# ebartrum/lightning_gan_zoo

Measured on AMD Instinct MI355X. Metric: images/sec (G+D step) at 64x64 bs=128/GPU, higher is better.
Workload: dtype f32; 1 GPU; dc_gan synthetic 64x64 bs=128/GPU, one optimizer cycle of 2 batches (Lightning alternation + toggle), reference optimizer, fp32; key=dc_gan_bs128, global_batch=128, parallelism=dp1, images_counted=2*bs*n_gpus per step (every batch of the cycle)

## Files before the change

### lightning_gan_zoo_amd/csrc/gz_igemm2.h

```cpp
#pragma once
#include "gz_igemm_core.h"

namespace gz {

constexpr int STAGES2 = 3;
constexpr uint32_t SOFF_OOB = 0x80000000u;

template <int WM_, int WN_, int TN_, int OCC_, int TM_ = 4>
struct TileCfg2 {
    static constexpr int WM = WM_, WN = WN_, TM = TM_, TN = TN_, OCC = OCC_;
    static constexpr int BM = WM * TM * 32, BN = WN * TN * 32;
    static_assert(WM * WN == 4, "4 wavefronts per workgroup, one per SIMD");
};

template <int BN>
struct MContigB2 {
    static_assert(BN == 64 || BN == 128 || BN == 256, "piece mapping");
    using Params = typename MContigLoader<BN>::Params;
    static constexpr int LD = BN, ROWS = BK;
    static constexpr int PIECES = BK * BN / 256 / 4;
    static constexpr int RPP = 256 / BN;
    __amdgpu_buffer_rsrc_t rsrc;
    uint32_t voff, ldb;
    int wave;
    __device__ __forceinline__ void init(const Params& p, int tile, int y, int tid) {
        rsrc = make_rsrc(p.base + (long long)y * p.batch_stride, (uint32_t)p.K * p.ld * 4u);
        const int lane = tid & 63;
        wave = __builtin_amdgcn_readfirstlane(tid >> 6);
        const int f = lane * 4, r = f / BN, col = f % BN;
        const int n = tile * BN + col;
        ldb = (uint32_t)p.ld * 4u;
        voff = n < p.MN ? (uint32_t)(r * p.ld + n) * 4u : OOB;
    }
    __device__ __forceinline__ void issue_piece(int kc, float* stage, int p, bool live) {
        const int piece = wave * PIECES + p;
        bload_lds16(rsrc, stage + piece * 256, voff, live ? (uint32_t)(kc * BK + piece * RPP) * ldb : SOFF_OOB);
    }
};

template <int BM>
struct ConvDgA2 {
    static_assert(BM == 256 || BM == 512, "whole 256-pixel pieces per LDS row");
    using Params = typename ConvDgALoader<BM, 4, 4, 2, 1>::Params;
    static constexpr int PPR = BM / 256;
    static constexpr int LD = BM + 4, ROWS = BK / 2, PIECES = 2 * PPR;
    static constexpr int ZERO_COL = BM;
    static constexpr bool ROWSHARE = true;
    __amdgpu_buffer_rsrc_t rsrc;
    uint32_t voff[2 * PPR];
    int wave, K, OHW, shift_half1;
    __device__ __forceinline__ void init(const Params& p, int tile, int phase, int tid) {
        const ConvShape& s = p.s;
        rsrc = make_rsrc(p.y, (uint32_t)s.N * s.K * s.OH * s.OW * 4u);
        const int lane = tid & 63;
        wave = __builtin_amdgcn_readfirstlane(tid >> 6);
        K = s.K; OHW = s.OH * s.OW;
        const int py = phase / 2, px = phase % 2;
        shift_half1 = (px + 1) / 2 - 1;
#pragma unroll
        for (int hb = 0; hb < PPR; ++hb) {
            const uint32_t m = (uint32_t)tile * BM + hb * 256 + lane * 4;
            const bool m_ok = m < (uint32_t)s.N * p.AH * p.AW;
            const uint32_t n = fdiv(m, p.div_ahw);
            const uint32_t pix = m - n * (uint32_t)(p.AH * p.AW);
            const uint32_t a = fdiv(pix, p.div_aw);
            const uint32_t b = pix - a * (uint32_t)p.AW;
#pragma unroll
            for (int ty = 0; ty < 2; ++ty) {
                const int oy = (int)a + (py + 1) / 2 - ty;
                const bool ok = m_ok && (unsigned)oy < (unsigned)s.OH;
                voff[ty * PPR + hb] = ok ? (n * (uint32_t)(s.K * OHW) + (uint32_t)(oy * s.OW) + b) * 4u : OOB;
            }
        }
    }
    __device__ __forceinline__ int frag_shift(int half) const { return half ? shift_half1 : shift_half1 + 1; }
    __device__ __forceinline__ void issue_piece(int kc, float* stage, int p, bool live) {
        const int kol = kc * (BK / 4) + wave;
        bload_lds16(rsrc, stage + (wave * 2 + p / PPR) * LD + (p % PPR) * 256, voff[p],
                    (live && kol < K) ? (uint32_t)kol * (uint32_t)OHW * 4u : SOFF_OOB);
    }
};

template <int BM, int OWC>
struct ConvFwdA2 {
    static_assert(BM == 256 && BM % OWC == 0 && OWC >= 2, "piece mapping");
    using Params = typename ConvFwdALoader<BM, 4, 4, 2, 1>::Params;
    static constexpr int LD = BM, ROWS = BK / 2, PIECES = 2;
    static constexpr int OW_C = OWC;
    static constexpr int EXTRA = (6 * OWC + 4 + 3) & ~3;
    static constexpr bool FWDROWS = true;
    __amdgpu_buffer_rsrc_t rsrc;
    uint32_t voff[2];
    int wave, HW, C;
    __device__ __forceinline__ void init(const Params& p, int tile, int y, int tid) {
        const ConvShape& s = p.s;
        rsrc = make_rsrc(p.x, (uint32_t)(s.N * s.C * s.H * s.W) * 4u);
        const int lane = tid & 63;
        wave = __builtin_amdgcn_readfirstlane(tid >> 6);
        HW = s.H * s.W; C = s.C;
#pragma unroll
        for (int q = 0; q < 2; ++q) {
            const int f = ((wave * 2 + q) * 64 + lane) * 4;
            const int seg = f / (8 * OWC), rem = f - seg * 8 * OWC;
            const int ky = rem / (2 * OWC), col = rem - ky * 2 * OWC;
            const uint32_t m = (uint32_t)tile * BM + seg * OWC;
            const bool m_ok = m < (uint32_t)s.N * s.OH * s.OW;
            const uint32_t n = fdiv(m, p.div_ohw);
            const uint32_t oy = fdiv(m - n * (uint32_t)(s.OH * s.OW), p.div_ow);
            const int iy = (int)oy * 2 - 1 + ky;
            const bool ok = m_ok && (unsigned)iy < (unsigned)s.H;
            voff[q] = ok ? (n * (uint32_t)(s.C * HW) + (uint32_t)(iy * s.W + col)) * 4u : OOB;
        }
    }
    static constexpr int ZERO = ROWS * LD;
    __device__ __forceinline__ void frag(int m_local, int half, int& even, int& odd) const {
        const int seg = m_local / OWC, ox = m_local - seg * OWC;
        const int base = seg * 8 * OWC + 2 * ox - 1 + half;
        even = (half == 0 && ox == 0) ? ZERO : base;
        odd = (half == 1 && ox == OWC - 1) ? ZERO : base + 2;
    }
    __device__ __forceinline__ void issue_piece(int kc, float* stage, int p, bool live) {
        bload_lds16(rsrc, stage + (wave * 2 + p) * 256, voff[p], (live && kc < C) ? (uint32_t)kc * (uint32_t)HW * 4u : SOFF_OOB);
    }
};

template <class Geo_>
struct TapGatherA2 {
    using Geo = Geo_;
    using Params = typename Geo::Params;
    static constexpr int BM = Geo::BM, LD = BM, ROWS = BK;
    static constexpr int G = BM / 64;
    static constexpr int PIECES = BK * G / 4;
    Geo geo;
    __amdgpu_buffer_rsrc_t rsrc;
    uint32_t vbase[G], veff[G];
    typename Geo::Pix pix[G];
    int wave, blocks, last_tap, last_kc, cb;
    uint32_t tap_soff;
    __device__ __forceinline__ void init(const Params& p, int tile, int y, int tid) {
        rsrc = geo.init(p, y);
        const int lane = tid & 63;
        wave = __builtin_amdgcn_readfirstlane(tid >> 6);
        blocks = round_bk(geo.chans) / BK;
        last_tap = -1; last_kc = -1; cb = 0; tap_soff = 0;
#pragma unroll
        for (int g = 0; g < G; ++g) {
            vbase[g] = geo.locate(p, (uint32_t)tile * BM + g * 64 + lane, pix[g]);
            veff[g] = OOB;
        }
    }
    __device__ __forceinline__ void issue_piece(int kc, float* stage, int p, bool live) {
        if (p == 0) {
            int tap = last_tap;
            if (kc == last_kc + 1 && last_kc >= 0) {
                cb += BK;
                if (cb >= blocks * BK) { cb = 0; ++tap; }
            } else {
                tap = kc / blocks;
// ... 125 lines not shown
template <int BM>
struct PlaneA2 {
    static_assert(BM % 256 == 0, "whole 256-pixel pieces per LDS row");
    struct Params {
        const float* base;
        int CH, HW, M;
        FastDiv div_hw;
    };
    static constexpr int LD = BM, ROWS = BK;
    static constexpr int PPR = BM / 256;
    static constexpr int PIECES = BK * PPR / 4;
    __amdgpu_buffer_rsrc_t rsrc;
    uint32_t voff[PPR], plane;
    int wave, CH;
    __device__ __forceinline__ void init(const Params& p, int tile, int y, int tid) {
        rsrc = make_rsrc(p.base, (uint32_t)(p.M / p.HW) * (uint32_t)p.CH * (uint32_t)p.HW * 4u);
        const int lane = tid & 63;
        wave = __builtin_amdgcn_readfirstlane(tid >> 6);
        CH = p.CH;
        plane = (uint32_t)p.HW * 4u;
#pragma unroll
        for (int g = 0; g < PPR; ++g) {
            const uint32_t m = (uint32_t)tile * BM + g * 256 + 4 * lane;
            const uint32_t n = fdiv(m, p.div_hw);
            voff[g] = m < (uint32_t)p.M ? (n * (uint32_t)(p.CH * p.HW) + (m - n * (uint32_t)p.HW)) * 4u : OOB;
        }
    }
    __device__ __forceinline__ void issue_piece(int kc, float* stage, int p, bool live) {
        const int row = wave * 4 + p / PPR, g = p % PPR;
        const int c = kc * BK + row;
        bload_lds16(rsrc, stage + row * LD + g * 256, voff[g], (live && c < CH) ? (uint32_t)c * plane : SOFF_OOB);
    }
};

#ifdef GZ2_STAMPS
__device__ unsigned long long gz2_stamps[8192 * 8];
#define GZ2_STAMP(var) const unsigned long long var = __builtin_amdgcn_s_memtime()
#else
#define GZ2_STAMP(var)
#endif

#ifndef GZ2_EXP_NOP
#define GZ2_NOP ""
#else
#define GZ2_NOP "s_nop 1\n\t"
#endif
template <int OFF>
__device__ __forceinline__ float lds_rd(uint32_t byte_addr) {
    float v;
    asm volatile("ds_read_b32 %0, %1 offset:%2" : "=v"(v) : "v"(byte_addr), "n"(OFF) : "memory");
    return v;
}
__device__ __forceinline__ void mfma_row(f32x16 (&c)[4], float a, const float (&b)[4]) {
    asm volatile(GZ2_NOP
                 "v_mfma_f32_32x32x2_f32 %0, %5, %4, %0\n\t"
                 "v_mfma_f32_32x32x2_f32 %1, %6, %4, %1\n\t"
                 "v_mfma_f32_32x32x2_f32 %2, %7, %4, %2\n\t"
                 "v_mfma_f32_32x32x2_f32 %3, %8, %4, %3"
                 : "+a"(c[0]), "+a"(c[1]), "+a"(c[2]), "+a"(c[3])
                 : "v"(a), "v"(b[0]), "v"(b[1]), "v"(b[2]), "v"(b[3]));
}
__device__ __forceinline__ void mfma_row(f32x16 (&c)[2], float a, const float (&b)[2]) {
    asm volatile(GZ2_NOP
                 "v_mfma_f32_32x32x2_f32 %0, %3, %2, %0\n\t"
                 "v_mfma_f32_32x32x2_f32 %1, %4, %2, %1"
                 : "+a"(c[0]), "+a"(c[1])
                 : "v"(a), "v"(b[0]), "v"(b[1]));
}
__device__ __forceinline__ void mfma_row(f32x16 (&c)[1], float a, const float (&b)[1]) {
    asm volatile(GZ2_NOP
                 "v_mfma_f32_32x32x2_f32 %0, %2, %1, %0"
                 : "+a"(c[0])
                 : "v"(a), "v"(b[0]));
}
__device__ __forceinline__ void mfma_one(f32x16& c, float a, float b) {
    asm volatile(GZ2_NOP
                 "v_mfma_f32_32x32x2_f32 %0, %2, %1, %0"
                 : "+a"(c)
                 : "v"(a), "v"(b));
}
__device__ __forceinline__ void mfma_row_mn(f32x16 (&c)[4], float a, const float (&b)[4]) {
    asm volatile(GZ2_NOP
                 "v_mfma_f32_32x32x2_f32 %0, %4, %5, %0\n\t"
                 "v_mfma_f32_32x32x2_f32 %1, %4, %6, %1\n\t"
                 "v_mfma_f32_32x32x2_f32 %2, %4, %7, %2\n\t"
                 "v_mfma_f32_32x32x2_f32 %3, %4, %8, %3"
                 : "+a"(c[0]), "+a"(c[1]), "+a"(c[2]), "+a"(c[3])
                 : "v"(a), "v"(b[0]), "v"(b[1]), "v"(b[2]), "v"(b[3]));
}
__device__ __forceinline__ void mfma_row_mn(f32x16 (&c)[2], float a, const float (&b)[2]) {
    asm volatile(GZ2_NOP
                 "v_mfma_f32_32x32x2_f32 %0, %2, %3, %0\n\t"
                 "v_mfma_f32_32x32x2_f32 %1, %2, %4, %1"
                 : "+a"(c[0]), "+a"(c[1])
                 : "v"(a), "v"(b[0]), "v"(b[1]));
}
__device__ __forceinline__ void lgkm_done(float (&a)[4], float (&b)[4]) {
    asm volatile("s_waitcnt lgkmcnt(0)" : "+v"(a[0]), "+v"(a[1]), "+v"(a[2]), "+v"(a[3]), "+v"(b[0]), "+v"(b[1]), "+v"(b[2]), "+v"(b[3]));
}
__device__ __forceinline__ void lgkm_done(float (&a)[4], float (&b)[2]) {
    asm volatile("s_waitcnt lgkmcnt(0)" : "+v"(a[0]), "+v"(a[1]), "+v"(a[2]), "+v"(a[3]), "+v"(b[0]), "+v"(b[1]));
}
__device__ __forceinline__ void lgkm_done(float (&a)[2], float (&b)[4]) {
    asm volatile("s_waitcnt lgkmcnt(0)" : "+v"(a[0]), "+v"(a[1]), "+v"(b[0]), "+v"(b[1]), "+v"(b[2]), "+v"(b[3]));
}
__device__ __forceinline__ void lgkm_done(float (&a)[4], float (&b)[1]) {
    asm volatile("s_waitcnt lgkmcnt(0)" : "+v"(a[0]), "+v"(a[1]), "+v"(a[2]), "+v"(a[3]), "+v"(b[0]));
}

template <class AL, class = void>
struct a_extra_of { static constexpr int value = 0; };
template <class AL>
struct a_extra_of<AL, std::void_t<decltype(AL::EXTRA)>> { static constexpr int value = AL::EXTRA; };
template <class AL>
constexpr int igemm2_a_extra() { return a_extra_of<AL>::value; }
template <class AL, class = void>
struct fwd_ow_of { static constexpr int value = 1; };
template <class AL>
struct fwd_ow_of<AL, std::void_t<decltype(AL::OW_C)>> { static constexpr int value = AL::OW_C; };
template <class AL>
constexpr int fwd_ow() { return fwd_ow_of<AL>::value; }

template <class AL>
constexpr int mode_count_of() {
    if constexpr (is_dualmode<AL>::value) return AL::MODES;
    else return 1;
}
template <class AL>
constexpr bool mode_plain_of(int m, int S) {
    if constexpr (is_dualmode<AL>::value) return AL::step_plain(m, S);
    else return false;
}
template <class AL>
constexpr unsigned mode_mask_of(int m, int S) {
    if constexpr (is_dualmode<AL>::value) return AL::step_mask(m, S);
    else return 0xFu;
}
template <class AL>
constexpr int ksteps_of() {
    if constexpr (is_dualmode<AL>::value) return AL::KSTEPS;
    else return BK / 2;
}
template <class AL>
constexpr int step_arow_of(int m, int S) {
    if constexpr (is_dualmode<AL>::value) return AL::step_arow(m, S);
    else return S;
}
template <class AL>
constexpr int step_brow_of(int m, int S) {
    if constexpr (is_dualmode<AL>::value) return AL::step_brow(m, S);
    else return 2 * S;
}

template <class Cfg, class AL, class BL, int KG>
constexpr int igemm2_ring_floats() {
    return ((STAGES2 * (AL::ROWS * AL::LD + igemm2_a_extra<AL>() + BL::ROWS * BL::LD) + 63) / 64) * 64;
}

template <class Cfg, class AL, class BL, class Epi, int KG = 1>
__global__ __launch_bounds__(NT * KG, KG == 1 ? Cfg::OCC : 2) void igemm2_kernel(typename AL::Params pa, typename BL::Params pb,
                                                                              typename Epi::Params pe, GridMap gm) {
    constexpr int LDA = AL::LD, LDB = BL::LD;
    constexpr int TM = Cfg::TM, TN = Cfg::TN;
    static_assert((TM == 4 || (TM == 2 && is_dualmode<AL>::value)) && (TN == 1 || TN == 2 || TN == 4),
                  "fragment registers of the hand-ordered k-step");
    static_assert(KG == 1 || (KG == 2 && TN <= 2), "two wave groups: the parked accumulators must fit the LDS");
    constexpr bool RS = is_rowshare<AL>::value;
    constexpr bool FR = is_fwdrows<AL>::value;
    constexpr bool DM = is_dualmode<AL>::value;
    static_assert(!DM || (RS && KG == 1 && (TN == 2 || TN == 4)), "multi-mode: row-shared loader, phases in the accumulator blocks");
    constexpr int A_EXTRA = igemm2_a_extra<AL>();
    constexpr int A_ELEMS = AL::ROWS * LDA + A_EXTRA, B_ELEMS = BL::ROWS * LDB;
    constexpr int STAGE = A_ELEMS + B_ELEMS;
    constexpr int PAD = 16;
    extern __shared__ __attribute__((aligned(16))) float smem2[];
    const int kg = KG == 1 ? 0 : __builtin_amdgcn_readfirstlane((int)threadIdx.x >> 8);
    float* const ring = smem2 + PAD + kg * igemm2_ring_floats<Cfg, AL, BL, KG>();
    GZ2_STAMP(st0);
#ifdef GZ2_STAMPS
    const unsigned long long sr0 = __builtin_amdgcn_s_memrealtime();
    unsigned long long st1 = st0, st2 = st0;
#endif

    const int tid = KG == 1 ? (int)threadIdx.x : ((int)threadIdx.x & (NT - 1));
    const int nwg = gridDim.x;
    int bid = blockIdx.x;
    if (gm.stagger > 0 && bid < 512 && blockIdx.z == 0) {
        const unsigned hw = __builtin_amdgcn_s_getreg(((4 - 1) << 11) | (16 << 6) | 4);
        if (hw & 1u) {
            const unsigned long long t_end = __builtin_amdgcn_s_memtime() + (unsigned long long)gm.stagger;
            while (__builtin_amdgcn_s_memtime() < t_end) __builtin_amdgcn_s_sleep(64);
        }
    }
    int y;
    if (gm.var_chunks) {
        const int tiles = gm.tiles_m * gm.tiles_n;
        y = gm.phase_order[bid / tiles];
        bid %= tiles;
    } else {
        if (!gm.no_swizzle) {
            const int q = nwg >> 3, rr = nwg & 7, x = bid & 7, i = bid >> 3;
            bid = (x < rr ? x * (q + 1) : rr * (q + 1) + (x - rr) * q) + i;
        }
        y = bid % gm.ny;
        bid /= gm.ny;
    }
    const int tile_n = bid % gm.tiles_n;
    const int tile_m = bid / gm.tiles_n;
    const int z = blockIdx.z;
    const int kcA = z * gm.chunks_per_split;
    const int kcB = min(gm.var_chunks ? gm.phase_chunks[y] : gm.chunks, kcA + gm.chunks_per_split);
    if (gm.slab && gm.var_chunks && kcA >= kcB) return;
    int kc0 = kcA, kc1 = kcB, kend = kcB;
    if constexpr (KG == 2) {
        const int h = (kcB - kcA + 1) >> 1;
        kc0 = kcA + kg * h;
        kend = kc0 + h;
        kc1 = min(kcB, kend);
    }

    AL al;
    BL bl;
    al.init(pa, tile_m, y, tid);
    bl.init(pb, tile_n, y, tid);

    f32x16 acc[TM][TN];
#pragma unroll
    for (int i = 0; i < TM; ++i)
#pragma unroll
        for (int j = 0; j < TN; ++j)
#pragma unroll
            for (int r = 0; r < 16; ++r) acc[i][j][r] = 0.f;

    const int lane = tid & 63, wave = __builtin_amdgcn_readfirstlane(tid >> 6);
    const int wm = wave / Cfg::WN, wn = wave % Cfg::WN;
    const int half = lane >> 5, l32 = lane & 31;
    const uint32_t lds0 = (uint32_t)(uintptr_t)(__attribute__((address_space(3))) float*)ring;
    uint32_t a_addr[TM];
#pragma unroll
    for (int i = 0; i < TM; ++i)
        a_addr[i] = lds0 + (uint32_t)(B_ELEMS + half * (RS ? 0 : LDA) + wm * TM * 32 + i * 32 + l32) * 4u;
    if constexpr (RS) {
        const int sh = al.frag_shift(half);
#pragma unroll
        for (int i = 0; i < TM; ++i) {
            const int b = (tile_m * Cfg::BM + wm * TM * 32 + i * 32 + l32) % pa.AW;
            const bool zero = (sh < 0 && b == 0) || (sh > 0 && b == pa.AW - 1);
            a_addr[i] = zero ? lds0 + (uint32_t)(B_ELEMS + AL::ZERO_COL) * 4u : a_addr[i] + (uint32_t)(sh * 4);
        }
        if (tid < STAGES2 * AL::ROWS * 4) {
            const int st = tid / (AL::ROWS * 4), q = tid % (AL::ROWS * 4);
            ring[st * STAGE + B_ELEMS + (q >> 2) * LDA + AL::ZERO_COL + (q & 3)] = 0.f;
        }
    }
    uint32_t a_addrB[TM];
    if constexpr (DM) {
#pragma unroll
        for (int i = 0; i < TM; ++i) {
            const int b = (tile_m * Cfg::BM + wm * TM * 32 + i * 32 + l32) % pa.AW;
            a_addrB[i] = lds0 + (uint32_t)(B_ELEMS + half * LDA + (b == 0 ? AL::ZERO_COL : wm * TM * 32 + i * 32 + l32 - 1)) * 4u;
        }
    }
    uint32_t a_odd[TM];
    if constexpr (FR) {
#pragma unroll
        for (int i = 0; i < TM; ++i) {
            int e, o;
            al.frag(wm * TM * 32 + i * 32 + l32, half, e, o);
            a_addr[i] = lds0 + (uint32_t)(B_ELEMS + e) * 4u;
            a_odd[i] = lds0 + (uint32_t)(B_ELEMS + o) * 4u;
        }
        for (int q = tid; q < STAGES2 * A_EXTRA; q += NT)
            ring[(q / A_EXTRA) * STAGE + B_ELEMS + AL::ZERO + q % A_EXTRA] = 0.f;
    }
    const uint32_t b_addr = lds0 + (uint32_t)(half * LDB + wn * TN * 32 + l32) * 4u;

    constexpr int NPA = AL::PIECES, NPB = BL::PIECES, NP = NPA + NPB, STEPS = ksteps_of<AL>();
    static_assert(STEPS == 8 || STEPS == 12, "k-steps per chunk");
    constexpr int PPS = (NP + STEPS - 1) / STEPS;
    static_assert(PPS <= 4 && NP < 64, "pieces are spread over the k-step's four MFMA rows; vmcnt is 6 bits");
    auto issue_piece = [&](int kc, int st, int p, bool live) {
#ifdef GZ2_EXP_NODMA
        if (kc >= kc0 + 2) return;
#endif
#ifdef GZ2_EXP_SAMECHUNK
        if (kc >= kc0 + 2) kc = kc0;
#endif
        float* sb = ring + st * STAGE;
        if (p < NPA) al.issue_piece(kc, sb + B_ELEMS, p, live);
        else bl.issue_piece(kc, sb, p - NPA, live);
    };
    auto fetch_m = [&](auto Sc, auto Mc, uint32_t so, float (&af)[TM], float (&bf)[TN]) {
        constexpr int S = decltype(Sc)::value, MD = decltype(Mc)::value;
        constexpr bool PL = mode_plain_of<AL>(MD, S);
        constexpr unsigned MK = mode_mask_of<AL>(MD, S);
        constexpr int AO = LDA * step_arow_of<AL>(MD, S) * 4, BO = step_brow_of<AL>(MD, S) * LDB * 4;
#pragma unroll
        for (int i = 0; i < TM; ++i) af[i] = lds_rd<AO>((PL ? a_addrB[i] : a_addr[i]) + so);
        if constexpr ((MK & 1u) != 0) bf[0] = lds_rd<BO>(b_addr + so);
        if constexpr (TN >= 2 && (MK & 2u) != 0) bf[1] = lds_rd<BO + 128>(b_addr + so);
        if constexpr (TN == 4 && (MK & 4u) != 0) bf[2] = lds_rd<BO + 256>(b_addr + so);
        if constexpr (TN == 4 && (MK & 8u) != 0) bf[3] = lds_rd<BO + 384>(b_addr + so);
    };
    auto fetch_first = [&](int kc, uint32_t so, float (&af)[TM], float (&bf)[TN]) {
        if constexpr (DM) {
            if (al.mode_of(kc) == 0) fetch_m(std::integral_constant<int, 0>{}, std::integral_constant<int, 0>{}, so, af, bf);
            else fetch_m(std::integral_constant<int, 0>{}, std::integral_constant<int, 1>{}, so, af, bf);
        }
    };
    auto fetch = [&](auto Sc, uint32_t so, float (&af)[TM], float (&bf)[TN]) {
        constexpr int S = decltype(Sc)::value;
        constexpr int AO = (RS ? LDA : 2 * LDA) * S * 4, BO = 2 * S * LDB * 4;
#ifdef GZ2_EXP_NOFETCH
        if (so != 0xFFFFFFFFu) return;
#endif
        if constexpr (FR) {
            constexpr int FO = (S >> 1) * 2 * fwd_ow<AL>() * 4;
            af[0] = lds_rd<FO>(((S & 1) ? a_odd[0] : a_addr[0]) + so);
            af[1] = lds_rd<FO>(((S & 1) ? a_odd[1] : a_addr[1]) + so);
            af[2] = lds_rd<FO>(((S & 1) ? a_odd[2] : a_addr[2]) + so);
            af[3] = lds_rd<FO>(((S & 1) ? a_odd[3] : a_addr[3]) + so);
        } else {
            af[0] = lds_rd<AO>(a_addr[0] + so);
            af[1] = lds_rd<AO>(a_addr[1] + so);
            af[2] = lds_rd<AO>(a_addr[2] + so);
            af[3] = lds_rd<AO>(a_addr[3] + so);
        }
        {
        bf[0] = lds_rd<BO>(b_addr + so);
        if constexpr (TN >= 2) bf[1] = lds_rd<BO + 128>(b_addr + so);
        if constexpr (TN == 4) {
            bf[2] = lds_rd<BO + 256>(b_addr + so);
            bf[3] = lds_rd<BO + 384>(b_addr + so);
        }
        }
    };
    auto mask = [&](float (&)[TM]) {};

    if (kcA < kcB) {
#pragma unroll
        for (int p = 0; p < NP; ++p) issue_piece(kc0, 0, p, kc0 < kc1);
#pragma unroll
        for (int p = 0; p < NP; ++p) issue_piece(kc0 + 1, 1, p, kc0 + 1 < kc1);
#ifdef GZ2_EXP_NO_LGKM_PROLOGUE
        asm volatile("s_waitcnt vmcnt(%0)" ::"n"(NP) : "memory");
#else
        asm volatile("s_waitcnt vmcnt(%0) lgkmcnt(0)" ::"n"(NP) : "memory");
#endif
        __builtin_amdgcn_s_barrier();
#ifdef GZ2_STAMPS
        st1 = __builtin_amdgcn_s_memtime();
#endif
        float af[2][TM], bf[2][TN];
#ifdef GZ2_STEP_STAMPS
        unsigned long long step_cyc[8] = {0, 0, 0, 0, 0, 0, 0, 0}, step_t = __builtin_amdgcn_s_memtime();
#endif
        if constexpr (DM) {
#pragma unroll
            for (int q = 0; q < 2; ++q)
#pragma unroll
                for (int j = 0; j < TN; ++j) bf[q][j] = 0.f;
            fetch_first(kc0, 0u, af[0], bf[0]);
        } else {
            fetch(std::integral_constant<int, 0>{}, 0u, af[0], bf[0]);
        }
        lgkm_done(af[0], bf[0]);
        mask(af[0]);
        int stage = 0;
        auto run_chunks = [&](int k_from, int k_to, auto Mc) {
        for (int kc = k_from; kc < k_to; ++kc) {
            int s1 = stage + 1; if (s1 >= STAGES2) s1 -= STAGES2;
            int s2 = s1 + 1; if (s2 >= STAGES2) s2 -= STAGES2;
            const uint32_t so = (uint32_t)(stage * STAGE * 4), sno = (uint32_t)(s1 * STAGE * 4);
            const bool more = kc + 2 < kc1;
            auto kstep = [&](auto Sc) {
                constexpr int S = decltype(Sc)::value;
                constexpr int MD = decltype(Mc)::value;
                constexpr int c = S & 1, n = c ^ 1;
                auto mfma_row = [&](f32x16 (&cc)[TN], float a, const float (&b)[TN]) {
                    if constexpr (DM) {
                        constexpr unsigned MK = mode_mask_of<AL>(MD, S);
                        if constexpr (MK == (TN == 4 ? 15u : 3u)) gz::mfma_row(cc, a, b);
                        else {
                            if constexpr ((MK & 1u) != 0) gz::mfma_one(cc[0], a, b[0]);
                            if constexpr (TN >= 2 && (MK & 2u) != 0) gz::mfma_one(cc[1], a, b[1]);
                            if constexpr (TN == 4 && (MK & 4u) != 0) gz::mfma_one(cc[2], a, b[2]);
                            if constexpr (TN == 4 && (MK & 8u) != 0) gz::mfma_one(cc[3], a, b[3]);
                        }
                    } else gz::mfma_row(cc, a, b);
                };
                auto fetch_same = [&](auto S2c, uint32_t o, float (&fa)[TM], float (&fb)[TN]) {
                    if constexpr (DM) fetch_m(S2c, Mc, o, fa, fb);
                    else fetch(S2c, o, fa, fb);
                };
                auto pieces = [&](auto Rowc) {
                    constexpr int row = decltype(Rowc)::value;
                    constexpr int r = PPS == 1 ? (row == 1 ? 0 : -1) : row;
                    constexpr int q = S * PPS + r;
                    if constexpr (r >= 0 && r < PPS && q < NP) issue_piece(kc + 2, s2, q, more);
                };
                if constexpr (S + 1 < STEPS) {
                    fetch_same(std::integral_constant<int, S + 1>{}, so, af[n], bf[n]);
                    mfma_row(acc[0], af[c][0], bf[c]);
                    pieces(std::integral_constant<int, 0>{});
                    mfma_row(acc[1], af[c][1], bf[c]);
                    pieces(std::integral_constant<int, 1>{});
                    if constexpr (TM == 4) mfma_row(acc[2], af[c][2], bf[c]);
                    pieces(std::integral_constant<int, 2>{});
                    if constexpr (TM == 4) mfma_row(acc[3], af[c][3], bf[c]);
                    pieces(std::integral_constant<int, 3>{});
                } else {
                    mfma_row(acc[0], af[c][0], bf[c]);
                    pieces(std::integral_constant<int, 0>{});
                    if constexpr (TM == 4) mfma_row(acc[1], af[c][1], bf[c]);
                    pieces(std::integral_constant<int, 1>{});
                    pieces(std::integral_constant<int, 2>{});
                    pieces(std::integral_constant<int, 3>{});
#ifndef GZ2_EXP_NOVMWAIT
                    asm volatile("s_waitcnt vmcnt(%0)" ::"n"(NP) : "memory");
#endif
#ifndef GZ2_EXP_NOBARRIER
                    __builtin_amdgcn_s_barrier();
#endif
                    if constexpr (DM) fetch_first(kc + 1, sno, af[n], bf[n]);
                    else fetch(std::integral_constant<int, 0>{}, sno, af[n], bf[n]);
                    if constexpr (TM == 4) {
                        mfma_row(acc[2], af[c][2], bf[c]);
                        mfma_row(acc[3], af[c][3], bf[c]);
                    } else {
                        mfma_row(acc[1], af[c][1], bf[c]);
                    }
                }
#ifdef GZ2_STEP_STAMPS
                {
                    const unsigned long long t = __builtin_amdgcn_s_memtime();
                    step_cyc[S] += t - step_t;
                    step_t = t;
                }
#endif
                lgkm_done(af[n], bf[n]);
                mask(af[n]);
            };
            kstep(std::integral_constant<int, 0>{});
            kstep(std::integral_constant<int, 1>{});
            kstep(std::integral_constant<int, 2>{});
            kstep(std::integral_constant<int, 3>{});
            kstep(std::integral_constant<int, 4>{});
            kstep(std::integral_constant<int, 5>{});
            kstep(std::integral_constant<int, 6>{});
            kstep(std::integral_constant<int, 7>{});
            if constexpr (STEPS == 12) {
                kstep(std::integral_constant<int, 8>{});
                kstep(std::integral_constant<int, 9>{});
                kstep(std::integral_constant<int, 10>{});
                kstep(std::integral_constant<int, 11>{});
            }
            stage = s1;
        }
        };
        if constexpr (DM) {
            run_chunks(kc0, min(kend, al.bound[0]), std::integral_constant<int, 0>{});
            run_chunks(max(kc0, al.bound[0]), kend, std::integral_constant<int, 1>{});
        } else {
            run_chunks(kc0, kend, std::integral_constant<int, 0>{});
        }
        asm volatile("s_waitcnt vmcnt(0)\n\ts_nop 15\n\ts_nop 15" ::: "memory");
#ifdef GZ2_STAMPS
        st2 = __builtin_amdgcn_s_memtime();
#endif
#ifdef GZ2_STEP_STAMPS
        if (tid == 0 && blockIdx.x < 64)
            for (int q = 0; q < 8; ++q) gz2_stamps[(size_t)(8192 - 64 + blockIdx.x) * 8 + q] = step_cyc[q];
#endif
    }

    if constexpr (KG == 2) {
        __syncthreads();
        float* const park = smem2;
        if (kg == 1) {
#pragma unroll
            for (int i = 0; i < TM; ++i)
#pragma unroll
                for (int j = 0; j < TN; ++j)
#pragma unroll
                    for (int r = 0; r < 16; ++r) park[((i * TN + j) * 16 + r) * NT + tid] = acc[i][j][r];
        }
        __syncthreads();
        if (kg == 1) return;
#pragma unroll
        for (int i = 0; i < TM; ++i)
#pragma unroll
            for (int j = 0; j < TN; ++j)
#pragma unroll
                for (int r = 0; r < 16; ++r) acc[i][j][r] += park[((i * TN + j) * 16 + r) * NT + tid];
    }
#ifdef GZ2_EXP_NOSTORE
    if (acc[0][0][0] == 123456.789f)
#endif
    if (gm.slab)
        store_slab<Epi::SWAP, TM, TN>(gm, acc, tile_m * Cfg::BM + wm * TM * 32, tile_n * Cfg::BN + wn * TN * 32, lane,
                                      gm.var_chunks ? gm.phase_slab0[y] + z : y * (int)gridDim.z + z);
    else
        Epi::template store<TM, TN>(pe, acc, tile_m * Cfg::BM + wm * TM * 32, tile_n * Cfg::BN + wn * TN * 32,
                                    lane, y, z);
#ifdef GZ2_STAMPS
    asm volatile("s_waitcnt vmcnt(0)" ::: "memory");
    if (tid == 0 && blockIdx.x < 8192) {
        unsigned long long* o = gz2_stamps + (size_t)blockIdx.x * 8;
        o[0] = st0; o[1] = st1; o[2] = st2; o[3] = __builtin_amdgcn_s_memtime();
        o[4] = sr0; o[5] = __builtin_amdgcn_s_memrealtime(); o[6] = kc1 - kc0; o[7] = TM * TN;
    }
#endif
}

template <class Cfg, class AL, class BL, class Epi>
__global__ __launch_bounds__(NT, Cfg::OCC) void igemm2r_kernel(typename AL::Params pa, typename BL::Params pb,
                                                               typename Epi::Params pe, GridMap gm) {
    constexpr int LDA = AL::LD, LDB = BL::LD;
    constexpr int TM = Cfg::TM, TN = Cfg::TN;
    static_assert(TM == 4 && (TN == 2 || TN == 4) && !Epi::SWAP, "fragment registers of the hand-ordered k-step");
    constexpr int A_ELEMS = BK * LDA, B_ELEMS = BK * LDB;
    constexpr int STAGE = A_ELEMS + B_ELEMS;
    extern __shared__ __attribute__((aligned(16))) float smem2[];
    float* const ring = smem2;

    const int tid = threadIdx.x;
    const int nwg = gridDim.x;
    int bid = blockIdx.x;
    if (!gm.no_swizzle) {
        const int q = nwg >> 3, rr = nwg & 7, x = bid & 7, i = bid >> 3;
        bid = (x < rr ? x * (q + 1) : rr * (q + 1) + (x - rr) * q) + i;
    }
    const int y = bid % gm.ny;
    bid /= gm.ny;
    const int tile_n = bid % gm.tiles_n;
    const int tile_m = bid / gm.tiles_n;
    const int z = blockIdx.z;
    const int kc0 = z * gm.chunks_per_split;
    const int kc1 = min(gm.chunks, kc0 + gm.chunks_per_split);

    AL al;
    BL bl;
    al.init(pa, tile_m, y, tid);
    bl.init(pb, tile_n, y, tid);

    f32x16 acc[TM][TN];
#pragma unroll
    for (int i = 0; i < TM; ++i)
#pragma unroll
        for (int j = 0; j < TN; ++j)
#pragma unroll
            for (int r = 0; r < 16; ++r) acc[i][j][r] = 0.f;

    const int lane = tid & 63, wave = __builtin_amdgcn_readfirstlane(tid >> 6);
    const int wm = wave / Cfg::WN, wn = wave % Cfg::WN;
    const int half = lane >> 5, l32 = lane & 31;
    const uint32_t lds0 = (uint32_t)(uintptr_t)(__attribute__((address_space(3))) float*)ring;
    const uint32_t a_addr = lds0 + (uint32_t)(B_ELEMS + half * LDA + wm * TM * 32 + l32) * 4u;
    const uint32_t b_addr = lds0 + (uint32_t)(half * LDB + wn * TN * 32 + l32) * 4u;
    constexpr int STEPS = BK / 2;
    auto fetch = [&](auto Sc, uint32_t so, float (&af)[TM], float (&bf)[TN]) {
        constexpr int S = decltype(Sc)::value;
        constexpr int AO = 2 * LDA * S * 4, BO = 2 * LDB * S * 4;
        af[0] = lds_rd<AO>(a_addr + so);
        af[1] = lds_rd<AO + 128>(a_addr + so);
        af[2] = lds_rd<AO + 256>(a_addr + so);
        af[3] = lds_rd<AO + 384>(a_addr + so);
        bf[0] = lds_rd<BO>(b_addr + so);
        if constexpr (TN >= 2) bf[1] = lds_rd<BO + 128>(b_addr + so);
        if constexpr (TN == 4) {
            bf[2] = lds_rd<BO + 256>(b_addr + so);
            bf[3] = lds_rd<BO + 384>(b_addr + so);
        }
    };

    if (kc0 < kc1) {
        al.issue(kc0);
        bl.issue(kc0);
        al.commit(ring + B_ELEMS);
        bl.commit(ring);
        asm volatile("s_waitcnt lgkmcnt(0)" ::: "memory");
        __builtin_amdgcn_s_barrier();
        float af[2][TM], bf[2][TN];
        fetch(std::integral_constant<int, 0>{}, 0u, af[0], bf[0]);
        lgkm_done(af[0], bf[0]);
        int stage = 0;
        for (int kc = kc0; kc < kc1; ++kc) {
            const uint32_t so = (uint32_t)(stage * STAGE * 4), sno = (uint32_t)((stage ^ 1) * STAGE * 4);
            float* const nxt = ring + (stage ^ 1) * STAGE;
            const bool more = kc + 1 < kc1;
            auto kstep = [&](auto Sc) {
                constexpr int S = decltype(Sc)::value;
                constexpr int c = S & 1, n = c ^ 1;
                if constexpr (S == 0) {
                    if (more) {
                        al.issue(kc + 1);
                        bl.issue(kc + 1);
                    }
                }
                if constexpr (S + 1 < STEPS) {
                    fetch(std::integral_constant<int, S + 1>{}, so, af[n], bf[n]);
                    mfma_row_mn(acc[0], af[c][0], bf[c]);
                    mfma_row_mn(acc[1], af[c][1], bf[c]);
                    if constexpr (S == STEPS - 3) { if (more) al.commit(nxt + B_ELEMS); }
                    if constexpr (S == STEPS - 2) { if (more) bl.commit(nxt); }
                    mfma_row_mn(acc[2], af[c][2], bf[c]);
                    mfma_row_mn(acc[3], af[c][3], bf[c]);
                    lgkm_done(af[n], bf[n]);
                } else {
                    mfma_row_mn(acc[0], af[c][0], bf[c]);
                    mfma_row_mn(acc[1], af[c][1], bf[c]);
                    __builtin_amdgcn_s_barrier();
                    fetch(std::integral_constant<int, 0>{}, sno, af[n], bf[n]);
                    mfma_row_mn(acc[2], af[c][2], bf[c]);
                    mfma_row_mn(acc[3], af[c][3], bf[c]);
                    lgkm_done(af[n], bf[n]);
                }
            };
            kstep(std::integral_constant<int, 0>{});
            kstep(std::integral_constant<int, 1>{});
            kstep(std::integral_constant<int, 2>{});
            kstep(std::integral_constant<int, 3>{});
            kstep(std::integral_constant<int, 4>{});
            kstep(std::integral_constant<int, 5>{});
            kstep(std::integral_constant<int, 6>{});
// ... 213 lines not shown
        cond = (oy0 == 0 ? 1u : 0u) | ((int)oy0 + BL::ROWS_PER_CHUNK == s.OH ? 2u : 0u) | (ox0 == 0 ? 4u : 0u) |
               ((int)ox0 + CW == s.OW ? 8u : 0u);
    };
    auto issue_piece = [&](int st, int q) {
        float* sb = ring + st * STAGE;
        if (q < NPA) al.issue_piece(sb + B_ELEMS, q, soff_a);
        else bl.issue_piece(sb, q - NPA, soff_b, cond);
    };
    auto fetch_a = [&](auto Gc, uint32_t so, f32x4 (&af)[TM]) {
        constexpr int G = decltype(Gc)::value;
        af[0] = lds_rd4<0>(a_addr[G] + so);
        af[1] = lds_rd4<32 * BK * 4>(a_addr[G] + so);
        af[2] = lds_rd4<64 * BK * 4>(a_addr[G] + so);
        af[3] = lds_rd4<96 * BK * 4>(a_addr[G] + so);
    };
    auto fetch_b = [&](auto Sc, uint32_t so, float (&bf)[TN]) {
        constexpr int S = decltype(Sc)::value;
        constexpr int BO = ((S >> 2) * BL::GOFF + (S & 3) * BL::TOFF) * 4;
        bf[0] = lds_rd<BO>(b_addr[0] + so);
        bf[1] = lds_rd<BO>(b_addr[1] + so);
    };

    if (kc0 < kc1) {
        locate(kc0, true);
#pragma unroll
        for (int q = 0; q < NP; ++q) issue_piece(0, q);
        locate(kc0 + 1, kc0 + 1 < kc1);
#pragma unroll
        for (int q = 0; q < NP; ++q) issue_piece(1, q);
        asm volatile("s_waitcnt vmcnt(%0)" ::"n"(NP) : "memory");
        __builtin_amdgcn_s_barrier();
        f32x4 af[2][TM];
        float bf[2][TN];
        fetch_a(std::integral_constant<int, 0>{}, 0u, af[0]);
        fetch_b(std::integral_constant<int, 0>{}, 0u, bf[0]);
        lgkm_done(af[0], bf[0]);
        int stage = 0;
        for (int kc = kc0; kc < kc1; ++kc) {
            int s1 = stage + 1; if (s1 >= STAGES2) s1 -= STAGES2;
            int s2 = s1 + 1; if (s2 >= STAGES2) s2 -= STAGES2;
            const uint32_t so = (uint32_t)(stage * STAGE * 4), sno = (uint32_t)(s1 * STAGE * 4);
            locate(kc + 2, kc + 2 < kc1);
            auto kstep = [&](auto Sc) {
                constexpr int S = decltype(Sc)::value;
                constexpr int c = S & 1, n = c ^ 1, g = S >> 2, t = S & 3;
                if constexpr (S + 1 < STEPS) {
                    fetch_b(std::integral_constant<int, S + 1>{}, so, bf[n]);
                    if constexpr (S == 0) fetch_a(std::integral_constant<int, 1>{}, so, af[1]);
                    mfma_row_mn(acc[0], af[g][0][t], bf[c]);
                    mfma_row_mn(acc[1], af[g][1][t], bf[c]);
                    if constexpr (S < NP) issue_piece(s2, S);
                    mfma_row_mn(acc[2], af[g][2][t], bf[c]);
                    mfma_row_mn(acc[3], af[g][3][t], bf[c]);
                    if constexpr (S == 0) lgkm_done(af[1], bf[n]);
                    else lgkm_done(bf[n]);
                } else {
                    mfma_row_mn(acc[0], af[g][0][t], bf[c]);
                    mfma_row_mn(acc[1], af[g][1][t], bf[c]);
                    if constexpr (S < NP) issue_piece(s2, S);
                    asm volatile("s_waitcnt vmcnt(%0)" ::"n"(NP) : "memory");
                    __builtin_amdgcn_s_barrier();
                    fetch_b(std::integral_constant<int, 0>{}, sno, bf[n]);
                    fetch_a(std::integral_constant<int, 0>{}, sno, af[0]);
                    mfma_row_mn(acc[2], af[g][2][t], bf[c]);
                    mfma_row_mn(acc[3], af[g][3][t], bf[c]);
                    lgkm_done(af[0], bf[n]);
                }
            };
            kstep(std::integral_constant<int, 0>{});
            kstep(std::integral_constant<int, 1>{});
            kstep(std::integral_constant<int, 2>{});
            kstep(std::integral_constant<int, 3>{});
            kstep(std::integral_constant<int, 4>{});
            kstep(std::integral_constant<int, 5>{});
            kstep(std::integral_constant<int, 6>{});
            kstep(std::integral_constant<int, 7>{});
            stage = s1;
        }
        asm volatile("s_waitcnt vmcnt(0)\n\ts_nop 15\n\ts_nop 15" ::: "memory");
    }
    Epi::template store<TM, TN>(pe, acc, tile_m * Cfg::BM + wm * TM * 32, tile_n * Cfg::BN + wn * TN * 32, lane, 0, z);
}

template <class Cfg, class BL>
constexpr size_t igemm2w_lds_bytes() {
    return (size_t)STAGES2 * (WgDyA2<Cfg::BM>::ELEMS + BL::ELEMS) * 4;
}

template <class Cfg, class BL, class Epi>
inline int launch_igemm2w(const Wg2Params& p, const typename Epi::Params& pe, int M, int N, int K, int splits,
                          hipStream_t stream) {
    GridMap gm;
    gm.no_swizzle = knobs().no_xcd_swizzle;
    gm.var_chunks = 0;
    gm.slab = nullptr;
    gm.slab_m = M;
    gm.slab_n = N;
    gm.tiles_m = (M + Cfg::BM - 1) / Cfg::BM;
    gm.tiles_n = (N + Cfg::BN - 1) / Cfg::BN;
    gm.chunks = (K + BK - 1) / BK;
    if (splits < 1) splits = 1;
    gm.chunks_per_split = (gm.chunks + splits - 1) / splits;
    int nz = (gm.chunks + gm.chunks_per_split - 1) / gm.chunks_per_split;
    if (nz < 1) nz = 1;
    gm.ny = 1;
    gm.stagger = 0;
    for (int i = 0; i < 8; ++i) gm.phase_nz[i] = gm.phase_slab0[i] = 0;
    dim3 grid(gm.tiles_m * gm.tiles_n, 1, nz);
    constexpr size_t lds = igemm2w_lds_bytes<Cfg, BL>();
    static_assert(lds <= 80 * 1024, "two workgroups per CU");
    auto kern = igemm2w_kernel<Cfg, BL, Epi>;
    static bool attr_done = false;
    if (!attr_done) {
        if (hipFuncSetAttribute((const void*)kern, hipFuncAttributeMaxDynamicSharedMemorySize, (int)lds) != hipSuccess)
            return launch_status();
        attr_done = true;
    }
    hipLaunchKernelGGL(kern, grid, dim3(NT), lds, stream, p, pe, gm);
    return launch_status();
}

template <class Cfg, class AL, class BL, class Epi>
inline int launch_igemm2r(const typename AL::Params& pa, const typename BL::Params& pb, const typename Epi::Params& pe,
                          int M, int N, int K, int splits, hipStream_t stream) {
    GridMap gm;
    gm.no_swizzle = knobs().no_xcd_swizzle;
    gm.var_chunks = 0;
    gm.slab = nullptr;
    gm.slab_m = M;
    gm.slab_n = N;
    gm.tiles_m = (M + Cfg::BM - 1) / Cfg::BM;
    gm.tiles_n = (N + Cfg::BN - 1) / Cfg::BN;
    gm.chunks = (K + BK - 1) / BK;
    if (splits < 1) splits = 1;
    gm.chunks_per_split = (gm.chunks + splits - 1) / splits;
    int nz = (gm.chunks + gm.chunks_per_split - 1) / gm.chunks_per_split;
    if (nz < 1) nz = 1;
    gm.ny = 1;
    gm.stagger = 0;
    for (int i = 0; i < 8; ++i) gm.phase_nz[i] = gm.phase_slab0[i] = 0;
    dim3 grid(gm.tiles_m * gm.tiles_n, 1, nz);
    constexpr size_t lds = (size_t)2 * BK * (AL::LD + BL::LD) * 4;
    auto kern = igemm2r_kernel<Cfg, AL, BL, Epi>;
    static bool attr_done = false;
    if (!attr_done) {
        if (hipFuncSetAttribute((const void*)kern, hipFuncAttributeMaxDynamicSharedMemorySize, (int)lds) != hipSuccess)
            return launch_status();
        attr_done = true;
    }
    hipLaunchKernelGGL(kern, grid, dim3(NT), lds, stream, pa, pb, pe, gm);
    return launch_status();
}

template <class Cfg, class AL, class BL>
constexpr size_t igemm2_lds_bytes() {
    return (size_t)(STAGES2 * (AL::ROWS * AL::LD + igemm2_a_extra<AL>() + BL::ROWS * BL::LD) + 32) * 4;
}
template <class Cfg, class AL, class BL>
constexpr size_t igemm2_lds_bytes_kg2() {
    const size_t rings = (size_t)(2 * igemm2_ring_floats<Cfg, AL, BL, 2>() + 32) * 4;
    const size_t park = (size_t)Cfg::TM * Cfg::TN * 16 * NT * 4;
    return rings > park ? rings : park;
}

template <class T, class = void>
struct is_tapgather : std::false_type {};
template <class T>
struct is_tapgather<T, std::void_t<decltype(T::Geo::TAPGATHER)>> : std::true_type {};
template <class Cfg, class AL>
constexpr bool igemm2_kg2_built() {
    return Cfg::TN <= 2 && Cfg::WM * Cfg::WN == 4 && Cfg::WN == 2 && !is_dualmode<AL>::value &&
           (is_rowshare<AL>::value || is_fwdrows<AL>::value || is_tapgather<AL>::value);
}
inline bool igemm2_use_kg2(long long workgroups, int chunks_per_workgroup) {
    if (knobs().no_kg2) return false;
    return workgroups <= cus() && chunks_per_workgroup >= knobs().kg2_min_chunks;
}

template <class Cfg, class AL, class BL, class Epi>
inline int launch_igemm2(const typename AL::Params& pa, const typename BL::Params& pb, const typename Epi::Params& pe,
                         int M, int N, int K, int ny, int splits, hipStream_t stream, float* slab = nullptr,
                         const int* phase_chunks = nullptr) {
    static_assert(Epi::SWAP, "transposed accumulators (lanes along m)");
    GridMap gm;
    gm.no_swizzle = knobs().no_xcd_swizzle;
    gm.var_chunks = 0;
    if (phase_chunks && ny <= 8) {
        gm.var_chunks = 1;
        for (int i = 0; i < ny; ++i) {
            gm.phase_chunks[i] = phase_chunks[i];
            gm.phase_order[i] = i;
        }
        for (int i = 1; i < ny; ++i)
            for (int j = i; j > 0 && gm.phase_chunks[gm.phase_order[j]] > gm.phase_chunks[gm.phase_order[j - 1]]; --j) {
                int t = gm.phase_order[j];
                gm.phase_order[j] = gm.phase_order[j - 1];
                gm.phase_order[j - 1] = t;
            }
    }
    gm.slab = nullptr;
    gm.slab_m = M;
    gm.slab_n = N;
    gm.tiles_m = (M + Cfg::BM - 1) / Cfg::BM;
    gm.tiles_n = (N + Cfg::BN - 1) / Cfg::BN;
    gm.chunks = (K + BK - 1) / BK;
    if (splits < 1) splits = 1;
    gm.chunks_per_split = (gm.chunks + splits - 1) / splits;
    int nz = (gm.chunks + gm.chunks_per_split - 1) / gm.chunks_per_split;
    if (nz < 1) nz = 1;
    gm.ny = ny;
    dim3 grid(gm.tiles_m * gm.tiles_n * ny, 1, nz);
    const int stagger_pct = knobs().igemm2_stagger;
    gm.stagger = (Cfg::OCC == 2 && nz == 1 && grid.x >= 1536)
                     ? (int)((long long)gm.chunks * 8 * Cfg::TM * Cfg::TN * 64 * 2 * stagger_pct / 100) : 0;
    if (slab && nz > 1) gm.slab = slab;
    SlabMap sm;
    sm.var = gm.slab && gm.var_chunks;
    for (int i = 0, at = 0; i < 8; ++i) {
        int n = (sm.var && i < ny) ? (gm.phase_chunks[i] + gm.chunks_per_split - 1) / gm.chunks_per_split : 0;
        gm.phase_nz[i] = sm.nz[i] = n;
        gm.phase_slab0[i] = sm.slab0[i] = at;
        at += n;
    }
    const size_t lds_extra = (size_t)knobs().igemm2_lds;
    bool launched = false;
    if constexpr (igemm2_kg2_built<Cfg, AL>()) {
        if (igemm2_use_kg2((long long)grid.x * nz, gm.chunks_per_split)) {
            const size_t lds2 = igemm2_lds_bytes_kg2<Cfg, AL, BL>();
            auto kern2 = igemm2_kernel<Cfg, AL, BL, Epi, 2>;
            static bool attr2_done = false;
            if (!attr2_done) {
                if (hipFuncSetAttribute((const void*)kern2, hipFuncAttributeMaxDynamicSharedMemorySize, (int)lds2) != hipSuccess)
                    return launch_status();
                attr2_done = true;
            }
            hipLaunchKernelGGL(kern2, grid, dim3(2 * NT), lds2, stream, pa, pb, pe, gm);
            launched = true;
        }
    }
    if (!launched) {
    const size_t lds = igemm2_lds_bytes<Cfg, AL, BL>() + lds_extra;
    auto kern = igemm2_kernel<Cfg, AL, BL, Epi>;
    static bool attr_done = false;
    if (!attr_done) {
        if (hipFuncSetAttribute((const void*)kern, hipFuncAttributeMaxDynamicSharedMemorySize, (int)lds) != hipSuccess)
            return launch_status();
        attr_done = true;
    }
    hipLaunchKernelGGL(kern, grid, dim3(NT), lds, stream, pa, pb, pe, gm);
    }
    if (gm.slab) {
        const int fm = (M + 31) / 32, fn = (N + 31) / 32;
        if (nz > 16)
            hipLaunchKernelGGL((splitk_finish_kernel<Epi, 8>), dim3(fm * fn * ny), dim3(512), 0, stream, slab, nz, M, N,
                               pe, fn, ny, sm);
        else
            hipLaunchKernelGGL((splitk_finish_kernel<Epi, 4>), dim3(fm * fn * ny), dim3(NT), 0, stream, slab, nz, M, N, pe,
                               fn, ny, sm);
    }
    return launch_status();
}

}
```

Measured before the change: 44910 images/s.

## Deepen implicit-GEMM LDS ring and batch barriers per chunk group for small tiles

Makes the LDS prefetch ring depth a per-config constant instead of a fixed three stages. For BM=256 row-shared or forward-row loaders with narrow output width, TN=1 configs get four or six stages and TN=2 configs three. TN=1 configs also process two chunks per barrier interval, so more global loads are in flight and barriers are fewer. It uses more LDS per workgroup, which can cut occupancy (guarded by static asserts on the LDS budget), and it adds unrolled k-steps and wider vmcnt wait counts.

```diff
diff --git a/lightning_gan_zoo_amd/csrc/gz_igemm2.h b/lightning_gan_zoo_amd/csrc/gz_igemm2.h
--- a/lightning_gan_zoo_amd/csrc/gz_igemm2.h
+++ b/lightning_gan_zoo_amd/csrc/gz_igemm2.h
@@ -4,6 +4,24 @@
 namespace gz {
 
 constexpr int STAGES2 = 3;
+#ifndef GZ2_DEPTH_TN1_KG2
+#define GZ2_DEPTH_TN1_KG2 6
+#endif
+#ifndef GZ2_DEPTH_TN1_KG1
+#define GZ2_DEPTH_TN1_KG1 4
+#endif
+#ifndef GZ2_DEPTH_TN2_KG2
+#define GZ2_DEPTH_TN2_KG2 3
+#endif
+#ifndef GZ2_DEPTH_TN2_KG1
+#define GZ2_DEPTH_TN2_KG1 3
+#endif
+#ifndef GZ2_BARRIER_TN1_KG2
+#define GZ2_BARRIER_TN1_KG2 2
+#endif
+#ifndef GZ2_BARRIER_TN1_KG1
+#define GZ2_BARRIER_TN1_KG1 2
+#endif
 constexpr uint32_t SOFF_OOB = 0x80000000u;
 
 template <int WM_, int WN_, int TN_, int OCC_, int TM_ = 4>
@@ -435,10 +453,42 @@
     else return 2 * S;
 }
 
+constexpr size_t LDS_PER_CU = 160 * 1024;
+template <class AL, class BL>
+constexpr int igemm2_stage_floats() { return AL::ROWS * AL::LD + igemm2_a_extra<AL>() + BL::ROWS * BL::LD; }
+template <class Cfg, class AL, class BL, int KG>
+constexpr size_t igemm2_lds_bytes_at(int depth) {
+    if (KG == 1) return (size_t)(depth * igemm2_stage_floats<AL, BL>() + 32) * 4;
+    const size_t rings = (size_t)(2 * ((depth * igemm2_stage_floats<AL, BL>() + 63) / 64 * 64) + 32) * 4;
+    const size_t park = (size_t)Cfg::TM * Cfg::TN * 16 * NT * 4;
+    return rings > park ? rings : park;
+}
+template <class Cfg, class AL, class BL, int KG>
+constexpr bool igemm2_tunable() {
+    return Cfg::BM == 256 && (is_rowshare<AL>::value || is_fwdrows<AL>::value) && !is_dualmode<AL>::value &&
+           fwd_ow<AL>() < 64;
+}
+template <class Cfg, class AL, class BL, int KG>
+constexpr int igemm2_interval() {
+    if (igemm2_tunable<Cfg, AL, BL, KG>() && Cfg::TN == 1) return KG == 2 ? GZ2_BARRIER_TN1_KG2 : GZ2_BARRIER_TN1_KG1;
+    return 1;
+}
+template <class Cfg, class AL, class BL, int KG>
+constexpr int igemm2_depth() {
+    if (igemm2_tunable<Cfg, AL, BL, KG>()) {
+        if (Cfg::TN == 1) return KG == 2 ? GZ2_DEPTH_TN1_KG2 : GZ2_DEPTH_TN1_KG1;
+        if (Cfg::TN == 2) return KG == 2 ? GZ2_DEPTH_TN2_KG2 : GZ2_DEPTH_TN2_KG1;
+    }
+    return STAGES2;
+}
 template <class Cfg, class AL, class BL, int KG>
 constexpr int igemm2_ring_floats() {
-    return ((STAGES2 * (AL::ROWS * AL::LD + igemm2_a_extra<AL>() + BL::ROWS * BL::LD) + 63) / 64) * 64;
-}
+    return ((igemm2_depth<Cfg, AL, BL, KG>() * igemm2_stage_floats<AL, BL>() + 63) / 64) * 64;
+}
+template <class Cfg, class AL, class BL>
+constexpr size_t igemm2_lds_bytes() { return igemm2_lds_bytes_at<Cfg, AL, BL, 1>(igemm2_depth<Cfg, AL, BL, 1>()); }
+template <class Cfg, class AL, class BL>
+constexpr size_t igemm2_lds_bytes_kg2() { return igemm2_lds_bytes_at<Cfg, AL, BL, 2>(igemm2_depth<Cfg, AL, BL, 2>()); }
 
 template <class Cfg, class AL, class BL, class Epi, int KG = 1>
 __global__ __launch_bounds__(NT * KG, KG == 1 ? Cfg::OCC : 2) void igemm2_kernel(typename AL::Params pa, typename BL::Params pb,
@@ -456,6 +506,14 @@
     constexpr int A_ELEMS = AL::ROWS * LDA + A_EXTRA, B_ELEMS = BL::ROWS * LDB;
     constexpr int STAGE = A_ELEMS + B_ELEMS;
     constexpr int PAD = 16;
+    constexpr int DEPTH = igemm2_depth<Cfg, AL, BL, KG>();
+    constexpr int BI = igemm2_interval<Cfg, AL, BL, KG>();
+    constexpr int GROUPS = DEPTH / BI;
+    static_assert(DEPTH % BI == 0 && (BI == 1 ? GROUPS >= 3 : GROUPS >= 2) && (BI == 1 || (BI == 2 && !DM)),
+                  "group t+GROUPS-1 lands in the stages group t-1 was read from");
+    static_assert(DEPTH == STAGES2 || (KG == 2 ? igemm2_lds_bytes_kg2<Cfg, AL, BL>()
+                                               : Cfg::OCC * igemm2_lds_bytes<Cfg, AL, BL>()) <= LDS_PER_CU,
+                  "workgroups per CU x LDS per workgroup");
     extern __shared__ __attribute__((aligned(16))) float smem2[];
     const int kg = KG == 1 ? 0 : __builtin_amdgcn_readfirstlane((int)threadIdx.x >> 8);
     float* const ring = smem2 + PAD + kg * igemm2_ring_floats<Cfg, AL, BL, KG>();
@@ -531,7 +589,8 @@
             const bool zero = (sh < 0 && b == 0) || (sh > 0 && b == pa.AW - 1);
             a_addr[i] = zero ? lds0 + (uint32_t)(B_ELEMS + AL::ZERO_COL) * 4u : a_addr[i] + (uint32_t)(sh * 4);
         }
-        if (tid < STAGES2 * AL::ROWS * 4) {
+        static_assert(DEPTH * AL::ROWS * 4 <= NT, "one pad float per thread");
+        if (tid < DEPTH * AL::ROWS * 4) {
             const int st = tid / (AL::ROWS * 4), q = tid % (AL::ROWS * 4);
             ring[st * STAGE + B_ELEMS + (q >> 2) * LDA + AL::ZERO_COL + (q & 3)] = 0.f;
         }
@@ -553,21 +612,24 @@
             a_addr[i] = lds0 + (uint32_t)(B_ELEMS + e) * 4u;
             a_odd[i] = lds0 + (uint32_t)(B_ELEMS + o) * 4u;
         }
-        for (int q = tid; q < STAGES2 * A_EXTRA; q += NT)
+        for (int q = tid; q < DEPTH * A_EXTRA; q += NT)
             ring[(q / A_EXTRA) * STAGE + B_ELEMS + AL::ZERO + q % A_EXTRA] = 0.f;
     }
     const uint32_t b_addr = lds0 + (uint32_t)(half * LDB + wn * TN * 32 + l32) * 4u;
 
     constexpr int NPA = AL::PIECES, NPB = BL::PIECES, NP = NPA + NPB, STEPS = ksteps_of<AL>();
-    static_assert(STEPS == 8 || STEPS == 12, "k-steps per chunk");
+    static_assert((STEPS == 8 || STEPS == 12) && (BI == 1 || STEPS == 8), "k-steps per chunk, per group 8, 12 or 16");
     constexpr int PPS = (NP + STEPS - 1) / STEPS;
-    static_assert(PPS <= 4 && NP < 64, "pieces are spread over the k-step's four MFMA rows; vmcnt is 6 bits");
+    static_assert(PPS <= 4 && (DEPTH - BI) * NP < 64,
+                  "pieces are spread over the k-step's four MFMA rows; vmcnt is 6 bits and DEPTH-BI chunks are in flight");
+    constexpr int NWAIT = (DEPTH - 2 * BI) * NP;
+    constexpr int GSTEPS = BI * STEPS;
     auto issue_piece = [&](int kc, int st, int p, bool live) {
 #ifdef GZ2_EXP_NODMA
-        if (kc >= kc0 + 2) return;
+        if (kc >= kc0 + DEPTH - BI) return;
 #endif
 #ifdef GZ2_EXP_SAMECHUNK
-        if (kc >= kc0 + 2) kc = kc0;
+        if (kc >= kc0 + DEPTH - BI) kc = kc0;
 #endif
         float* sb = ring + st * STAGE;
         if (p < NPA) al.issue_piece(kc, sb + B_ELEMS, p, live);
@@ -592,13 +654,14 @@
         }
     };
     auto fetch = [&](auto Sc, uint32_t so, float (&af)[TM], float (&bf)[TN]) {
-        constexpr int S = decltype(Sc)::value;
-        constexpr int AO = (RS ? LDA : 2 * LDA) * S * 4, BO = 2 * S * LDB * 4;
+        constexpr int S = decltype(Sc)::value % STEPS, JO = decltype(Sc)::value / STEPS * STAGE * 4;
+        constexpr int AO = (RS ? LDA : 2 * LDA) * S * 4 + JO, BO = 2 * S * LDB * 4 + JO;
+        static_assert(AO + 2 * LDA * 4 < 65536 && BO + 512 < 65536, "ds_read immediate offsets");
 #ifdef GZ2_EXP_NOFETCH
         if (so != 0xFFFFFFFFu) return;
 #endif
         if constexpr (FR) {
-            constexpr int FO = (S >> 1) * 2 * fwd_ow<AL>() * 4;
+            constexpr int FO = (S >> 1) * 2 * fwd_ow<AL>() * 4 + JO;
             af[0] = lds_rd<FO>(((S & 1) ? a_odd[0] : a_addr[0]) + so);
             af[1] = lds_rd<FO>(((S & 1) ? a_odd[1] : a_addr[1]) + so);
             af[2] = lds_rd<FO>(((S & 1) ? a_odd[2] : a_addr[2]) + so);
@@ -622,13 +685,13 @@
 
     if (kcA < kcB) {
 #pragma unroll
-        for (int p = 0; p < NP; ++p) issue_piece(kc0, 0, p, kc0 < kc1);
-#pragma unroll
-        for (int p = 0; p < NP; ++p) issue_piece(kc0 + 1, 1, p, kc0 + 1 < kc1);
+        for (int d = 0; d < DEPTH - BI; ++d)
+#pragma unroll
+            for (int p = 0; p < NP; ++p) issue_piece(kc0 + d, d, p, kc0 + d < kc1);
 #ifdef GZ2_EXP_NO_LGKM_PROLOGUE
-        asm volatile("s_waitcnt vmcnt(%0)" ::"n"(NP) : "memory");
+        asm volatile("s_waitcnt vmcnt(%0)" ::"n"(NWAIT) : "memory");
 #else
-        asm volatile("s_waitcnt vmcnt(%0) lgkmcnt(0)" ::"n"(NP) : "memory");
+        asm volatile("s_waitcnt vmcnt(%0) lgkmcnt(0)" ::"n"(NWAIT) : "memory");
 #endif
         __builtin_amdgcn_s_barrier();
 #ifdef GZ2_STAMPS
@@ -636,7 +699,8 @@
 #endif
         float af[2][TM], bf[2][TN];
 #ifdef GZ2_STEP_STAMPS
-        unsigned long long step_cyc[8] = {0, 0, 0, 0, 0, 0, 0, 0}, step_t = __builtin_amdgcn_s_memtime();
+        unsigned long long step_cyc[STEPS] = {}, step_t = __builtin_amdgcn_s_memtime();
+        unsigned long long wait_cyc[2] = {0, 0};
 #endif
         if constexpr (DM) {
 #pragma unroll
@@ -651,11 +715,11 @@
         mask(af[0]);
         int stage = 0;
         auto run_chunks = [&](int k_from, int k_to, auto Mc) {
-        for (int kc = k_from; kc < k_to; ++kc) {
-            int s1 = stage + 1; if (s1 >= STAGES2) s1 -= STAGES2;
-            int s2 = s1 + 1; if (s2 >= STAGES2) s2 -= STAGES2;
-            const uint32_t so = (uint32_t)(stage * STAGE * 4), sno = (uint32_t)(s1 * STAGE * 4);
-            const bool more = kc + 2 < kc1;
+        for (int kc = k_from; kc < k_to; kc += BI) {
+            int s1 = stage + 1; if (s1 >= GROUPS) s1 -= GROUPS;
+            int s2 = stage - 1; if (s2 < 0) s2 += GROUPS;
+            const uint32_t so = (uint32_t)(stage * BI * STAGE * 4), sno = (uint32_t)(s1 * BI * STAGE * 4);
+            const bool more = kc + DEPTH - BI < kc1, more1 = kc + DEPTH - BI + 1 < kc1;
             auto kstep = [&](auto Sc) {
                 constexpr int S = decltype(Sc)::value;
                 constexpr int MD = decltype(Mc)::value;
@@ -680,9 +744,10 @@
                     constexpr int row = decltype(Rowc)::value;
                     constexpr int r = PPS == 1 ? (row == 1 ? 0 : -1) : row;
                     constexpr int q = S * PPS + r;
-                    if constexpr (r >= 0 && r < PPS && q < NP) issue_piece(kc + 2, s2, q, more);
+                    if constexpr (r >= 0 && r < PPS && q < BI * NP)
+                        issue_piece(kc + DEPTH - BI + q / NP, s2 * BI + q / NP, q % NP, q / NP == 0 ? more : more1);
                 };
-                if constexpr (S + 1 < STEPS) {
+                if constexpr (S + 1 < GSTEPS) {
                     fetch_same(std::integral_constant<int, S + 1>{}, so, af[n], bf[n]);
                     mfma_row(acc[0], af[c][0], bf[c]);
                     pieces(std::integral_constant<int, 0>{});
@@ -699,13 +764,26 @@
                     pieces(std::integral_constant<int, 1>{});
                     pieces(std::integral_constant<int, 2>{});
                     pieces(std::integral_constant<int, 3>{});
+#ifdef GZ2_STEP_STAMPS
+                    const unsigned long long tw0 = __builtin_amdgcn_s_memtime();
+#endif
 #ifndef GZ2_EXP_NOVMWAIT
-                    asm volatile("s_waitcnt vmcnt(%0)" ::"n"(NP) : "memory");
+                    asm volatile("s_waitcnt vmcnt(%0)" ::"n"(NWAIT) : "memory");
+#endif
+#ifdef GZ2_STEP_STAMPS
+                    const unsigned long long tw1 = __builtin_amdgcn_s_memtime();
 #endif
 #ifndef GZ2_EXP_NOBARRIER
                     __builtin_amdgcn_s_barrier();
 #endif
-                    if constexpr (DM) fetch_first(kc + 1, sno, af[n], bf[n]);
+#ifdef GZ2_STEP_STAMPS
+                    {
+                        const unsigned long long tw2 = __builtin_amdgcn_s_memtime();
+                        wait_cyc[0] += tw1 - tw0;
+                        wait_cyc[1] += tw2 - tw1;
+                    }
+#endif
+                    if constexpr (DM) fetch_first(kc + BI, sno, af[n], bf[n]);
                     else fetch(std::integral_constant<int, 0>{}, sno, af[n], bf[n]);
                     if constexpr (TM == 4) {
                         mfma_row(acc[2], af[c][2], bf[c]);
@@ -717,7 +795,7 @@
 #ifdef GZ2_STEP_STAMPS
                 {
                     const unsigned long long t = __builtin_amdgcn_s_memtime();
-                    step_cyc[S] += t - step_t;
+                    step_cyc[S % STEPS] += t - step_t;
                     step_t = t;
                 }
 #endif
@@ -732,11 +810,17 @@
             kstep(std::integral_constant<int, 5>{});
             kstep(std::integral_constant<int, 6>{});
             kstep(std::integral_constant<int, 7>{});
-            if constexpr (STEPS == 12) {
+            if constexpr (GSTEPS >= 12) {
                 kstep(std::integral_constant<int, 8>{});
                 kstep(std::integral_constant<int, 9>{});
                 kstep(std::integral_constant<int, 10>{});
                 kstep(std::integral_constant<int, 11>{});
+            }
+            if constexpr (GSTEPS == 16) {
+                kstep(std::integral_constant<int, 12>{});
+                kstep(std::integral_constant<int, 13>{});
+                kstep(std::integral_constant<int, 14>{});
+                kstep(std::integral_constant<int, 15>{});
             }
             stage = s1;
         }
@@ -754,6 +838,11 @@
 #ifdef GZ2_STEP_STAMPS
         if (tid == 0 && blockIdx.x < 64)
             for (int q = 0; q < 8; ++q) gz2_stamps[(size_t)(8192 - 64 + blockIdx.x) * 8 + q] = step_cyc[q];
+        if (tid == 0 && kg == 0 && blockIdx.x < 64) {
+            gz2_stamps[(size_t)(8192 - 128 + blockIdx.x) * 8 + 0] = wait_cyc[0];
+            gz2_stamps[(size_t)(8192 - 128 + blockIdx.x) * 8 + 1] = wait_cyc[1];
+            gz2_stamps[(size_t)(8192 - 128 + blockIdx.x) * 8 + 2] = (unsigned long long)(kend - kc0);
+        }
 #endif
     }
 
@@ -1273,17 +1362,6 @@
     return launch_status();
 }
 
-template <class Cfg, class AL, class BL>
-constexpr size_t igemm2_lds_bytes() {
-    return (size_t)(STAGES2 * (AL::ROWS * AL::LD + igemm2_a_extra<AL>() + BL::ROWS * BL::LD) + 32) * 4;
-}
-template <class Cfg, class AL, class BL>
-constexpr size_t igemm2_lds_bytes_kg2() {
-    const size_t rings = (size_t)(2 * igemm2_ring_floats<Cfg, AL, BL, 2>() + 32) * 4;
-    const size_t park = (size_t)Cfg::TM * Cfg::TN * 16 * NT * 4;
-    return rings > park ? rings : park;
-}
-
 template <class T, class = void>
 struct is_tapgather : std::false_type {};
 template <class T>
```

Result: faster. 45440 images/s (median of 6 runs) (+1.2%).
